# ComparativeGenomicsToolkit/paffy

Hardware: AMD Instinct MI355X
Metric: PAF records/sec (shatter+invert+trim pipe); % HBM roofline at 1/2/4/8 GPU (higher is better)
Workload: dtype u8/int64 (float32 identity predicate); 1 GPU; cfg3: 10M synthetic PAF records, mean 2k cigar ops, invert | trim | shatter; pipe=invert|trim|shatter, pipeline_contexts=2, stream_records=10000000, mean_cigar_ops=2048

## Files before the change

paffy_amd/csrc/flat_kernel.h:

```cpp
#ifndef PAFFY_FLAT_KERNEL_H_
#define PAFFY_FLAT_KERNEL_H_

#define FLAT_TILE 1024u
#define FLAT_TILE_SHIFT 10u
#define FLAT_CHUNK_PIECES 4u
#define FLAT_P_CAP 512u
#define FLAT_NO_CHUNK 0xffffffffu
#define FLAT_F_IRREG 1u
#define FLAT_F_NONPLAIN 2u

struct PieceSum {
    uint32_t cnt;
    uint32_t m, x;
    uint32_t ins, del;
    uint32_t rows;
    uint32_t extra;
    uint32_t text_end;
};
static_assert(sizeof(PieceSum) == 32, "two 16-byte stores");

struct FlatParams {
    const uint8_t *in;
    uint32_t in_len;
    const RecMeta *meta;
    const uint32_t *chunk_rec;
    uint32_t n_chunk_slots;
    const uint16_t *nd;
    PieceSum *sums;
    uint32_t *ops_mirror;
    DevInfo *info;
    uint32_t items_mode;
};

__device__ __forceinline__ uint32_t nondigit16(const uint4 &v) {
    const uint32_t w[4] = {v.x, v.y, v.z, v.w};
    uint32_t m = 0;
#pragma unroll
    for (int j = 0; j < 4; j++) {
        uint32_t nd = nondigit4(w[j]) >> 7;
        nd = (nd | (nd >> 7) | (nd >> 14) | (nd >> 21)) & 0xfu;
        m |= nd << (4 * j);
    }
    return m;
}
__device__ __forceinline__ uint32_t wave_fold_u32(uint32_t x) {
    x += dpp_mov_u32<DPP_ROW_SHR(1), 0xf, 0xf>(x);
    x += dpp_mov_u32<DPP_ROW_SHR(2), 0xf, 0xf>(x);
    x += dpp_mov_u32<DPP_ROW_SHR(4), 0xf, 0xf>(x);
    x += dpp_mov_u32<DPP_ROW_SHR(8), 0xf, 0xf>(x);
    x += dpp_mov_u32<DPP_BCAST15, 0xa, 0xf>(x);
    x += dpp_mov_u32<DPP_BCAST31, 0xc, 0xf>(x);
    return x;
}
__device__ __forceinline__ uint32_t wave_sum_u32(uint32_t v) { return wave_last_u32(wave_fold_u32(v)); }
__device__ __forceinline__ void wave_sum6_u32(uint32_t (&x)[6]) {
#define FLAT_FOLD_STEP(CTRL, RM)                                                  \
    _Pragma("unroll") for (int k = 0; k < 6; k++) x[k] += dpp_mov_u32<CTRL, RM, 0xf>(x[k]);
    FLAT_FOLD_STEP(DPP_ROW_SHR(1), 0xf)
    FLAT_FOLD_STEP(DPP_ROW_SHR(2), 0xf)
    FLAT_FOLD_STEP(DPP_ROW_SHR(4), 0xf)
    FLAT_FOLD_STEP(DPP_ROW_SHR(8), 0xf)
    FLAT_FOLD_STEP(DPP_BCAST15, 0xa)
    FLAT_FOLD_STEP(DPP_BCAST31, 0xc)
#undef FLAT_FOLD_STEP
#pragma unroll
    for (int k = 0; k < 6; k++) x[k] = wave_last_u32(x[k]);
}
__device__ __forceinline__ uint32_t uni(uint32_t x) { return (uint32_t)__builtin_amdgcn_readfirstlane((int)x); }
__device__ __forceinline__ uint32_t lane_val(uint32_t x, uint32_t l) { return (uint32_t)__builtin_amdgcn_readlane((int)x, (int)l); }

#define FLAT_PARSE_LDS (16u + FLAT_TILE + 2u * FLAT_P_CAP)
#define FLAT_PARSE_WAVES 4u
template <uint32_t MODE>
__global__ __launch_bounds__(64 * FLAT_PARSE_WAVES) void k_flat_parse(FlatParams F) {
    __shared__ __attribute__((aligned(16))) uint8_t smem[FLAT_PARSE_WAVES][FLAT_PARSE_LDS];
    const uint32_t lane = threadIdx.x & 63u, wave = uni(threadIdx.x >> 6);
    uint8_t *T = smem[wave];
    uint16_t *Pl = reinterpret_cast<uint16_t *>(T + 16u + FLAT_TILE);
    const uint32_t n_waves = gridDim.x * FLAT_PARSE_WAVES;
    for (uint32_t c = blockIdx.x * FLAT_PARSE_WAVES + wave; c < F.n_chunk_slots; c += n_waves) {
        const uint32_t rec = F.chunk_rec[c];
        if (rec == FLAT_NO_CHUNK) continue;
        const uint32_t cg_off = F.meta[rec].cg_off, cg_end = cg_off + F.meta[rec].cg_len;
        const uint32_t tile_first = cg_off >> FLAT_TILE_SHIFT;
        const uint32_t np = ((cg_end - 1u) >> FLAT_TILE_SHIFT) - tile_first + 1u;
        const uint32_t p0 = (c - ((tile_first >> 2) + rec)) * FLAT_CHUNK_PIECES, p1 = p0 + FLAT_CHUNK_PIECES < np ? p0 + FLAT_CHUNK_PIECES : np;
        PieceSum *const rec_sums = F.sums + (tile_first + rec);
        uint32_t tile = tile_first + p0;
        __builtin_amdgcn_wave_barrier();
        if (lane == 0) {
            uint4 h = make_uint4(0, 0, 0, 0);
            if (tile > 0) h = *reinterpret_cast<const uint4 *>(F.in + ((size_t)tile << FLAT_TILE_SHIFT) - 16u);
            *reinterpret_cast<uint4 *>(T) = h;
        }
        __builtin_amdgcn_wave_barrier();
        uint32_t n = 0;
        int32_t prev;
        uint32_t text_end = 0;
        if (p0 == 0) {
            prev = (int32_t)cg_off - 1 - (int32_t)(tile << FLAT_TILE_SHIFT);
        } else {
            uint32_t cnt = 0;
            {
                const uint32_t g = (tile_first << FLAT_TILE_SHIFT) + lane * 16u;
                uint4 v = make_uint4(0x30303030u, 0x30303030u, 0x30303030u, 0x30303030u);
                if (g < F.in_len) v = *reinterpret_cast<const uint4 *>(F.in + g);
                const uint32_t lo_b = cg_off > g ? (cg_off - g < 16u ? cg_off - g : 16u) : 0u;
                cnt = (uint32_t)__popc(nondigit16(v) & 0xffffu & ~((1u << lo_b) - 1u));
            }
            for (uint32_t t = tile_first + 1u + lane; t < tile; t += 64u) cnt += F.nd[t];
            n = wave_sum_u32(cnt);
            const uint4 h = *reinterpret_cast<const uint4 *>(T);
            const uint32_t hm = nondigit16(h);
            prev = hm ? (int32_t)(31 - __clz((int)hm)) - 16 : -17;
            text_end = (uint32_t)((int32_t)(tile << FLAT_TILE_SHIFT) + prev + 1 - (int32_t)cg_off);
        }
        uint16_t *dst = reinterpret_cast<uint16_t *>(F.ops_mirror + (cg_off >> 1));
        for (uint32_t p = p0; p < p1; p++, tile++) {
            const uint32_t t0 = tile << FLAT_TILE_SHIFT, g = t0 + lane * 16u;
            uint4 v = make_uint4(0, 0, 0, 0);
            if (g < F.in_len) v = *reinterpret_cast<const uint4 *>(F.in + g);
            *reinterpret_cast<uint4 *>(T + 16u + lane * 16u) = v;
            const uint32_t ndm = nondigit16(v);
            const uint32_t lo_b = cg_off > g ? (cg_off - g < 16u ? cg_off - g : 16u) : 0u;
            const uint32_t hi_b = cg_end < g + 16u ? (cg_end > g ? cg_end - g : 0u) : 16u;
            uint32_t opmask = ndm & (hi_b >= 16u ? 0xffffu : ((1u << hi_b) - 1u)) & ~((1u << lo_b) - 1u);
            uint32_t bad = (hi_b > lo_b && g + hi_b == cg_end && !((ndm >> (hi_b - 1u)) & 1u)) ? 1u : 0u;
            const uint32_t cnt = (uint32_t)__popc(opmask), inc = wave_incl_scan_u32(cnt), total = wave_last_u32(inc);
            uint32_t rank = inc - cnt;
            while (opmask) {
                const uint32_t j = (uint32_t)__ffs((int)opmask) - 1u;
                opmask &= opmask - 1u;
                if (rank < FLAT_P_CAP) Pl[rank] = (uint16_t)(lane * 16u + j);
                rank++;
            }
            if (total > FLAT_P_CAP) bad = 1u;
            __builtin_amdgcn_wave_barrier();
            const uint32_t top = total < FLAT_P_CAP ? total : FLAT_P_CAP;
            uint32_t acc_mx = 0, acc_id = 0, acc_re = 0, nonplain = 0;
            uint32_t before_first = (uint32_t)prev;
            for (uint32_t i = lane; i < top; i += 64u) {
                const uint32_t pos = Pl[i];
                const uint32_t before = (uint32_t)__builtin_amdgcn_update_dpp((int)before_first, (int)pos, 0x138 , 0xf, 0xf, false);
                before_first = lane_val(pos, 63);
                const uint32_t k = pos - before - 1u;
                const uint32_t a = 12u + pos, sh = a & 3u;
                const uint32_t *wp = reinterpret_cast<const uint32_t *>(T + (a - sh));
                const uint32_t d0 = wp[0], d1 = wp[1];
                const uint32_t hi = __builtin_amdgcn_alignbyte(d1, d0, sh);
                const uint32_t ch = (d1 >> (8u * sh)) & 0xffu;
                const uint32_t kk = k < 4u ? k : 4u;
                const uint32_t x = kk ? ((hi ^ 0x30303030u) & (0xffffffffu << (32u - 8u * kk))) : 0u;
                const uint32_t pr = ((x << 3) + (x << 1) + (x >> 8)) & 0x00ff00ffu;
                const uint32_t len = __umul24(pr & 0xffu, 100u) + (pr >> 16);
                const uint32_t dl = ch - 0x3du;
                const bool known = dl < 28u && ((0x08011081u >> dl) & 1u);
                const uint32_t code = (0x04001023u >> (dl & 0x1cu)) & 7u;
                const bool lead0 = kk >= 2u && ((hi >> (8u * (4u - kk))) & 0xffu) == (uint32_t)'0';
                bad |= ((k - 1u > 3u) | (len - 1u >= 8191u) | lead0 | !known) ? 1u : 0u;
                dst[n + i] = (uint16_t)((len << 3) | code);
                const uint32_t l16 = len & 0xffffu;
                acc_mx += l16 << (((0x16u >> code) & 1u) << 4);
                acc_id += (code == (uint32_t)OP_I ? l16 : 0u) + (code == (uint32_t)OP_D ? l16 << 16 : 0u);
                if (MODE == 2u) acc_re += (code == (uint32_t)OP_M ? 1u : 0u) + (code == (uint32_t)OP_I ? 1u << 16 : 0u);
                else acc_re += code == (uint32_t)OP_M ? 1u + ((MODE == 1u ? (len + 15u) >> 4 : kk - 1u) << 16) : 0u;
                nonplain |= code > (uint32_t)OP_D ? 1u : 0u;
            }
            uint32_t sums6[6] = {acc_mx & 0xffffu, acc_mx >> 16, acc_id & 0xffffu, acc_id >> 16, acc_re & 0xffffu, acc_re >> 16};
            wave_sum6_u32(sums6);
            const uint32_t s_m = sums6[0], s_x = sums6[1], s_i = sums6[2], s_d = sums6[3], s_r = sums6[4], s_e = sums6[5];
            const uint32_t flags = (__any(bad != 0) ? FLAT_F_IRREG : 0u) | (__any(nonplain != 0) ? FLAT_F_NONPLAIN : 0u);
            if (total) {
                const int32_t last = (int32_t)Pl[top - 1u];
                text_end = t0 + (uint32_t)last + 1u - cg_off;
                prev = last - (int32_t)FLAT_TILE;
            } else {
                prev -= (int32_t)FLAT_TILE;
                if (prev < -64) prev = -64;
            }
            if (lane == 0) {
                uint4 *o = reinterpret_cast<uint4 *>(rec_sums + p);
                o[0] = make_uint4(total | (flags << 16), s_m, s_x, s_i);
                o[1] = make_uint4(s_d, s_r, s_e, text_end);
            }
            n += total;
            __builtin_amdgcn_wave_barrier();
            if (lane == 63u) *reinterpret_cast<uint4 *>(T) = v;
            __builtin_amdgcn_wave_barrier();
        }
    }
}


struct FlatSizeParams {
    KParams P;
    PieceSum *sums;
    uint8_t *flat_done;
    uint32_t *defer;
};

struct FlatPre {
    uint32_t cnt, m, x, ins, del, rows, extra, text;
};
__device__ __forceinline__ FlatPre flat_sub(const FlatPre &a, const FlatPre &b) {
    FlatPre r;
    r.cnt = a.cnt - b.cnt; r.m = a.m - b.m; r.x = a.x - b.x; r.ins = a.ins - b.ins; r.del = a.del - b.del;
    r.rows = a.rows - b.rows; r.extra = a.extra - b.extra; r.text = a.text - b.text;
    return r;
}
__device__ __forceinline__ uint32_t flat_ld(const uint32_t *p) { return __hip_atomic_load(p, __ATOMIC_RELAXED, __HIP_MEMORY_SCOPE_AGENT); }

struct FlatRec {
    const PieceSum *ps;
    uint32_t np, n_ops;
    bool in_regs;
    FlatPre inc;
    const uint16_t *ops;
    bool want_text;
    bool extra_icount;

    __device__ __forceinline__ FlatPre piece_prefix(uint32_t j) const {
        FlatPre r;
        r.cnt = r.m = r.x = r.ins = r.del = r.rows = r.extra = r.text = 0;
        if (j == 0) return r;
        if (in_regs) {
            const uint32_t l = j - 1u;
            r.cnt = lane_val(inc.cnt, l); r.m = lane_val(inc.m, l); r.x = lane_val(inc.x, l); r.ins = lane_val(inc.ins, l);
            r.del = lane_val(inc.del, l); r.rows = lane_val(inc.rows, l); r.extra = lane_val(inc.extra, l); r.text = lane_val(inc.text, l);
        } else {
            const uint32_t *q = reinterpret_cast<const uint32_t *>(ps + (j - 1u));
            r.cnt = uni(flat_ld(q)); r.m = uni(flat_ld(q + 1)); r.x = uni(flat_ld(q + 2)); r.ins = uni(flat_ld(q + 3));
            r.del = uni(flat_ld(q + 4)); r.rows = uni(flat_ld(q + 5)); r.extra = uni(flat_ld(q + 6)); r.text = uni(flat_ld(q + 7));
        }
        return r;
    }
    __device__ __forceinline__ uint32_t piece_of(uint32_t r) const {
        if (in_regs) {
            const uint32_t lane = threadIdx.x & 63u;
            return (uint32_t)__popcll(__ballot(lane < np && inc.cnt <= r));
        }
        uint32_t lo = 0, hi = np;
        while (lo < hi) {
            const uint32_t mid = (lo + hi) >> 1;
            if (uni(flat_ld(&ps[mid].cnt)) <= r) lo = mid + 1u;
            else hi = mid;
        }
        return lo;
    }
    __device__ __forceinline__ FlatPre raw_prefix(uint32_t r) const {
        if (r >= n_ops) return piece_prefix(np);
        const uint32_t pc = piece_of(r);
        FlatPre a = piece_prefix(pc);
        if (a.cnt == r) return a;
        const uint32_t lane = threadIdx.x & 63u;
        uint32_t sm = 0, sx = 0, si = 0, sd = 0, sr = 0, se = 0, st = 0;
        for (uint32_t i = a.cnt + lane; i < r; i += 64u) {
            const uint32_t w = ops[i], len = w >> 3, code = w & 7u;
            const uint32_t is_m = 0u - ((0x9u >> code) & 1u);
            const uint32_t dg = (len >= 10u) + (len >= 100u) + (len >= 1000u);
            sm += len & is_m;
            sx += len & ~is_m;
            si += code == (uint32_t)OP_I ? len : 0u;
            sd += code == (uint32_t)OP_D ? len : 0u;
            sr += code == (uint32_t)OP_M ? 1u : 0u;
            se += extra_icount ? (code == (uint32_t)OP_I ? 1u : 0u) : (code == (uint32_t)OP_M ? dg : 0u);
            st += dg + 2u;
        }
        uint32_t sums6[6] = {sm, sx, si, sd, sr, se};
        wave_sum6_u32(sums6);
        a.m += sums6[0]; a.x += sums6[1]; a.ins += sums6[2]; a.del += sums6[3];
        a.rows += sums6[4]; a.extra += sums6[5];
        if (want_text) a.text += wave_sum_u32(st);
        a.cnt = r;
        return a;
    }
};

struct FlatView {
    uint32_t lo, n;
    bool rev, swp;
    FlatPre wlo, whi;
    uint32_t cut_m = 0, cut_x = 0;
    __device__ __forceinline__ uint32_t tm() const { return whi.m - wlo.m - cut_m; }
    __device__ __forceinline__ uint32_t tx() const { return whi.x - wlo.x - cut_x; }
    __device__ __forceinline__ uint32_t ins_v() const { return swp ? whi.del - wlo.del : whi.ins - wlo.ins; }
    __device__ __forceinline__ uint32_t del_v() const { return swp ? whi.ins - wlo.ins : whi.del - wlo.del; }
    __device__ __forceinline__ int64_t tq() const { return (int64_t)tm() + (int64_t)tx() - (int64_t)del_v(); }
    __device__ __forceinline__ int64_t tt() const { return (int64_t)tm() + (int64_t)tx() - (int64_t)ins_v(); }
};

struct FlatState {
    int64_t qlen, qs, qe, tlen, ts, te;
    bool same;
};
__device__ __forceinline__ void flat_invert(FlatState &s) {
    int64_t t;
    t = s.qs; s.qs = s.ts; s.ts = t;
    t = s.qe; s.qe = s.te; s.te = t;
    t = s.qlen; s.qlen = s.tlen; s.tlen = t;
}
__device__ __forceinline__ int flat_check(const FlatState &s, const FlatView &v) {
    if (s.qs < 0 || s.qs >= s.qlen) return PAFFY_ERR_CHECK_QSTART;
    if (s.qs > s.qe || s.qe > s.qlen) return PAFFY_ERR_CHECK_QEND;
    if (s.ts < 0 || s.ts >= s.tlen) return PAFFY_ERR_CHECK_TSTART;
    if (s.ts > s.te || s.te > s.tlen) return PAFFY_ERR_CHECK_TEND;
    if (v.tq() != s.qe - s.qs) return PAFFY_ERR_CHECK_CIGAR_Q;
    if (v.tt() != s.te - s.ts) return PAFFY_ERR_CHECK_CIGAR_T;
    return 0;
}

__device__ __forceinline__ bool flat_filter_pass(const KParams &P, const RecMeta &m, const FlatView &v) {
    const int64_t mm = v.tm(), mx = v.tx();
    const int64_t all = mm + mx;
    const int64_t ins = all - v.tt(), del = all - v.tq();
    const double identity = ratio_f32(mm, mm + (mx - ins - del));
    const double identity_with_gaps = ratio_f32(mm, all);
    const int64_t f_as = P.filter.min_alignment_score, f_cs = P.filter.min_chain_score, f_tl = P.filter.max_tile_level;
    const double f_id = P.filter.min_identity, f_idg = P.filter.min_identity_with_gaps;
    return m.score >= f_as && m.chain_score >= f_cs && (f_tl == -1 || m.tile_level <= f_tl) && identity >= f_id && identity_with_gaps >= f_idg;
}
__device__ __forceinline__ void flat_dropped(const KParams &P, uint8_t *flat_done, uint32_t rec) {
    RecPlan *dp = static_cast<RecPlan *>(P.rec_plan) + rec;
    flat_done[rec] = 1;
    P.status[rec] = (uint32_t)KLASS_LDS << 16;
    P.err_aux[rec] = 0;
    P.n_ops[rec] = 0;
    P.out_len[rec] = 0;
    P.out_rows[rec] = 0;
    dp->flags = 128u;
    dp->n = 0;
}

__device__ __forceinline__ void flat_stats(const KParams &P, uint32_t rec, const FlatView &v) {
    const uint32_t n_i = v.whi.extra - v.wlo.extra, n_other = (v.whi.cnt - v.wlo.cnt) - (v.whi.rows - v.wlo.rows);
    const uint32_t n_d = n_other - n_i;
    int64_t *o = P.rec_stats + 6ull * rec;
    o[0] = (int64_t)v.tm();
    o[1] = (int64_t)v.tx() - (int64_t)(v.whi.ins - v.wlo.ins) - (int64_t)(v.whi.del - v.wlo.del);
    o[2] = (int64_t)(v.swp ? n_d : n_i);
    o[3] = (int64_t)(v.swp ? n_i : n_d);
    o[4] = (int64_t)v.ins_v();
    o[5] = (int64_t)v.del_v();
}
__device__ __forceinline__ bool flat_ratio_lt(uint32_t num, uint32_t den, float thr_f, double thr) {
    const float nf = __uint2float_rn(num), df = __uint2float_rn(den);
    const float p = __fmul_rn(thr_f, df);
    if (nf < __fmul_rn(p, 0.999996f)) return true;
    if (nf > __fmul_rn(p, 1.000004f)) return false;
    return (double)__fdiv_rn(nf, df) < thr;
}
__device__ __forceinline__ bool flat_ratio_ge(uint32_t num, uint32_t den, float id_f, double idd) {
    const float nf = __uint2float_rn(num), df = __uint2float_rn(den);
    const float p = __fmul_rn(id_f, df);
    if (nf > __fmul_rn(p, 1.000004f)) return true;
    if (nf < __fmul_rn(p, 0.999996f)) return false;
    return (double)__fdiv_rn(nf, df) >= idd;
}

__device__ __forceinline__ void flat_trim_prefix(const FlatRec &R, FlatState &s, FlatView &v, float thr_f, float id_f, int64_t max_trim) {
    const double thr = (double)thr_f, idd = (double)id_f;
    const uint32_t lane = threadIdx.x & 63u;
    const uint32_t w_end = v.lo + v.n;
    const uint32_t nb = (R.np + 63u) >> 6;
    int32_t trim_idx = -1;
    uint32_t hit_m = 0, hit_x = 0;
    for (uint32_t bi = 0; bi < nb && trim_idx < 0; bi++) {
        const uint32_t b = v.rev ? bi : nb - 1u - bi;
        const uint32_t p = b * 64u + lane;
        uint32_t a_cnt = 0, a_m = 0, a_x = 0, b_cnt = 0, b_m = 0, b_x = 0;
        if (p < R.np) {
            if (R.in_regs) {
                b_cnt = R.inc.cnt; b_m = R.inc.m; b_x = R.inc.x;
            } else {
                const uint32_t *q = reinterpret_cast<const uint32_t *>(R.ps + p);
                b_cnt = flat_ld(q); b_m = flat_ld(q + 1); b_x = flat_ld(q + 2);
            }
        }
        if (R.in_regs) {
            a_cnt = dpp_mov_u32<0x138, 0xf, 0xf>(b_cnt); a_m = dpp_mov_u32<0x138, 0xf, 0xf>(b_m); a_x = dpp_mov_u32<0x138, 0xf, 0xf>(b_x);
        } else if (p > 0 && p < R.np) {
            const uint32_t *q = reinterpret_cast<const uint32_t *>(R.ps + (p - 1u));
            a_cnt = flat_ld(q); a_m = flat_ld(q + 1); a_x = flat_ld(q + 2);
        }
        if (a_cnt < v.lo) { a_cnt = v.lo; a_m = v.wlo.m; a_x = v.wlo.x; }
        if (a_cnt > w_end) { a_cnt = w_end; a_m = v.whi.m; a_x = v.whi.x; }
        if (b_cnt < v.lo) { b_cnt = v.lo; b_m = v.wlo.m; b_x = v.wlo.x; }
        if (b_cnt > w_end) { b_cnt = w_end; b_m = v.whi.m; b_x = v.whi.x; }
        const bool live = p < R.np && b_cnt > a_cnt;
        const uint32_t c_m = v.rev ? v.whi.m - b_m : a_m - v.wlo.m, c_x = v.rev ? v.whi.x - b_x : a_x - v.wlo.x;
        const uint32_t chunk_x = b_x - a_x;
        const bool may_hit = live && !(c_m > 0 && (double)c_m >= thr * 1.00001 * (double)(c_m + c_x + chunk_x)) &&
                             !(max_trim >= 0 && (int64_t)c_m + (int64_t)c_x > max_trim);
        unsigned long long flagged = __ballot(may_hit);
        while (flagged) {
            const uint32_t t = v.rev ? (uint32_t)__ffsll((long long)flagged) - 1u : 63u - (uint32_t)__clzll((long long)flagged);
            flagged &= ~(1ull << t);
            const uint32_t ra = lane_val(a_cnt, t), rb = lane_val(b_cnt, t);
            uint32_t pm = lane_val(c_m, t), px = lane_val(c_x, t);
            const uint32_t x_end = px + lane_val(chunk_x, t);
            const uint32_t vb = v.rev ? w_end - rb : ra - v.lo, ve = v.rev ? w_end - ra : rb - v.lo;
            int32_t hit = -1;
            for (uint32_t i0 = vb; i0 < ve; i0 += 64u) {
                if (i0 != vb && pm > 0 && (double)pm >= thr * 1.00001 * (double)(pm + x_end)) break;
                const uint32_t i = i0 + lane;
                uint32_t len = 0, code = 0;
                if (i < ve) {
                    const uint32_t w = R.ops[v.rev ? w_end - 1u - i : v.lo + i];
                    len = w >> 3;
                    code = w & 7u;
                }
                const uint32_t is_m = 0u - ((0x9u >> code) & 1u);
                const uint32_t im = wave_incl_scan_u32(len & is_m), ix = wave_incl_scan_u32(len & ~is_m);
                const uint32_t cm = pm + im, cx = px + ix;
                const bool ok = i < ve && !(max_trim >= 0 && (int64_t)(cm + cx) > max_trim) && flat_ratio_lt(cm, cm + cx, thr_f, thr);
                const unsigned long long hb = __ballot(ok);
                if (hb) {
                    const uint32_t hl = 63u - (uint32_t)__clzll((long long)hb);
                    hit = (int32_t)(i0 + hl);
                    hit_m = lane_val(cm, hl);
                    hit_x = lane_val(cx, hl);
                }
                pm += wave_last_u32(im);
                px += wave_last_u32(ix);
            }
            if (hit >= 0) {
                trim_idx = hit;
                break;
            }
        }
    }
    if (trim_idx < 0) return;
    uint32_t best = 0xffffffffu;
    {
        uint32_t pm = 0, px = 0;
        for (uint32_t i0 = 0; i0 <= (uint32_t)trim_idx && best == 0xffffffffu; i0 += 64u) {
            const uint32_t i = i0 + lane;
            uint32_t len = 0, code = 0;
            if (i <= (uint32_t)trim_idx) {
                const uint32_t w = R.ops[v.rev ? w_end - 1u - i : v.lo + i];
                len = w >> 3;
                code = w & 7u;
            }
            const uint32_t is_m = 0u - ((0x9u >> code) & 1u);
            const uint32_t vm = len & is_m, vx = len & ~is_m;
            const uint32_t im = wave_incl_scan_u32(vm), ix = wave_incl_scan_u32(vx);
            const uint32_t sm = hit_m - (pm + im - vm), sx = hit_x - (px + ix - vx);
            const bool ok = i <= (uint32_t)trim_idx && flat_ratio_ge(sm, sm + sx, id_f, idd);
            const unsigned long long hb = __ballot(ok);
            if (hb) best = i0 + (uint32_t)__ffsll((long long)hb) - 1u;
            pm += wave_last_u32(im);
            px += wave_last_u32(ix);
        }
    }
    const uint32_t count = best != 0xffffffffu ? best : (uint32_t)trim_idx + 1u;
    if (count == 0) return;
    const int64_t old_tt = v.tt(), old_tq = v.tq();
    {
        const FlatPre cut = R.raw_prefix(v.rev ? v.lo + v.n - count : v.lo + count);
        if (v.rev) {
            v.whi = cut;
        } else {
            v.wlo = cut;
            v.lo += count;
        }
    }
    v.n -= count;
    const int64_t d_t = old_tt - v.tt(), d_q = old_tq - v.tq();
    s.ts += d_t;
    if (s.same) s.qs += d_q;
    else s.qe -= d_q;
}

#define FLAT_F_ROW_PIECES 0x200000u
#define FLAT_F_COPY 0x400000u
#define FLAT_COPY_MAX (1u << 18)
#define FLAT_ROW_PIECES_BYTES 144u
struct LanePieceSink {
    uint32_t (*S)[256];
// ... 941 lines not shown
```

Before: 24.79 million records/s.

## Parse CIGAR tile with per-step ballots instead of LDS position list

Replaces the two-pass parse (scatter op positions into an LDS list, then re-read them per lane) with a single pass over 128-byte steps. Each lane examines two bytes, uses ballots and mbcnt to rank op terminators, and reads the preceding digit word directly from the tile in LDS. Lengths are decoded with udot4 and op length is inferred from leading non-digits. This removes the serial ffs loop and the LDS position buffer, at the cost of more intricate edge handling for capped tiles and adjacent ops, and it recomputes the last-op position from ballot masks.

```diff
diff --git a/paffy_amd/csrc/flat_kernel.h b/paffy_amd/csrc/flat_kernel.h
--- a/paffy_amd/csrc/flat_kernel.h
+++ b/paffy_amd/csrc/flat_kernel.h
@@ -69,14 +69,21 @@
 __device__ __forceinline__ uint32_t uni(uint32_t x) { return (uint32_t)__builtin_amdgcn_readfirstlane((int)x); }
 __device__ __forceinline__ uint32_t lane_val(uint32_t x, uint32_t l) { return (uint32_t)__builtin_amdgcn_readlane((int)x, (int)l); }
 
-#define FLAT_PARSE_LDS (16u + FLAT_TILE + 2u * FLAT_P_CAP)
+#define FLAT_PARSE_LDS (16u + FLAT_TILE)
 #define FLAT_PARSE_WAVES 4u
+#define FLAT_STEP 128u
+__device__ __forceinline__ uint64_t lanes_below(uint32_t n) { return n >= 64u ? ~0ull : (1ull << n) - 1ull; }
+__device__ __forceinline__ bool lane_bit(uint64_t m) { return __builtin_amdgcn_inverse_ballot_w64(m); }
+__device__ __forceinline__ uint32_t lanes_before(uint64_t m, uint32_t add) {
+    return __builtin_amdgcn_mbcnt_hi((uint32_t)(m >> 32), __builtin_amdgcn_mbcnt_lo((uint32_t)m, add));
+}
 template <uint32_t MODE>
 __global__ __launch_bounds__(64 * FLAT_PARSE_WAVES) void k_flat_parse(FlatParams F) {
     __shared__ __attribute__((aligned(16))) uint8_t smem[FLAT_PARSE_WAVES][FLAT_PARSE_LDS];
     const uint32_t lane = threadIdx.x & 63u, wave = uni(threadIdx.x >> 6);
     uint8_t *T = smem[wave];
-    uint16_t *Pl = reinterpret_cast<uint16_t *>(T + 16u + FLAT_TILE);
+    const uint32_t *lw = reinterpret_cast<const uint32_t *>(T + 8u + (lane >> 1) * 4u);
+    const uint32_t o8 = (lane & 1u) * 16u;
     const uint32_t n_waves = gridDim.x * FLAT_PARSE_WAVES;
     for (uint32_t c = blockIdx.x * FLAT_PARSE_WAVES + wave; c < F.n_chunk_slots; c += n_waves) {
         const uint32_t rec = F.chunk_rec[c];
@@ -97,6 +104,7 @@
         uint32_t n = 0;
         int32_t prev;
         uint32_t text_end = 0;
+        bool capped = false;
         if (p0 == 0) {
             prev = (int32_t)cg_off - 1 - (int32_t)(tile << FLAT_TILE_SHIFT);
         } else {
@@ -121,59 +129,101 @@
             uint4 v = make_uint4(0, 0, 0, 0);
             if (g < F.in_len) v = *reinterpret_cast<const uint4 *>(F.in + g);
             *reinterpret_cast<uint4 *>(T + 16u + lane * 16u) = v;
-            const uint32_t ndm = nondigit16(v);
-            const uint32_t lo_b = cg_off > g ? (cg_off - g < 16u ? cg_off - g : 16u) : 0u;
-            const uint32_t hi_b = cg_end < g + 16u ? (cg_end > g ? cg_end - g : 0u) : 16u;
-            uint32_t opmask = ndm & (hi_b >= 16u ? 0xffffu : ((1u << hi_b) - 1u)) & ~((1u << lo_b) - 1u);
-            uint32_t bad = (hi_b > lo_b && g + hi_b == cg_end && !((ndm >> (hi_b - 1u)) & 1u)) ? 1u : 0u;
-            const uint32_t cnt = (uint32_t)__popc(opmask), inc = wave_incl_scan_u32(cnt), total = wave_last_u32(inc);
-            uint32_t rank = inc - cnt;
-            while (opmask) {
-                const uint32_t j = (uint32_t)__ffs((int)opmask) - 1u;
-                opmask &= opmask - 1u;
-                if (rank < FLAT_P_CAP) Pl[rank] = (uint16_t)(lane * 16u + j);
-                rank++;
+            __builtin_amdgcn_wave_barrier();
+            const uint32_t lo = cg_off > t0 ? cg_off - t0 : 0u, hi = cg_end - t0 < FLAT_TILE ? cg_end - t0 : FLAT_TILE;
+            uint32_t bad = 0;
+            if (cg_end - t0 <= FLAT_TILE && hi > lo) bad = (uint32_t)T[16u + hi - 1u] - (uint32_t)'0' <= 9u ? 1u : 0u;
+            uint16_t *const dst_t = dst + n;
+            uint32_t acc_mx = 0, acc_id = 0, acc_re = 0, nonplain = 0;
+            uint32_t total = 0;
+            int32_t last = 0;
+            uint64_t e0 = 0, e1 = 0;
+            uint32_t eb = 0;
+#pragma unroll
+            for (uint32_t s = 0; s < FLAT_TILE / FLAT_STEP; s++) {
+                const uint32_t sb = s * FLAT_STEP;
+                if (hi <= sb || lo >= sb + FLAT_STEP) continue;
+                uint64_t in0 = ~0ull, in1 = ~0ull;
+                if (lo > sb || hi < sb + FLAT_STEP) {
+                    const uint32_t a = lo > sb ? lo - sb : 0u, b = hi - sb < FLAT_STEP ? hi - sb : FLAT_STEP;
+                    in0 = lanes_below((b + 1u) >> 1) & ~lanes_below((a + 1u) >> 1);
+                    in1 = lanes_below(b >> 1) & ~lanes_below(a >> 1);
+                }
+                const uint32_t w0 = lw[s * (FLAT_STEP / 4u)], w1 = lw[s * (FLAT_STEP / 4u) + 1u], w2 = lw[s * (FLAT_STEP / 4u) + 2u];
+                const uint32_t c0 = (w2 >> o8) & 0xffu, c1 = (w2 >> (o8 + 8u)) & 0xffu;
+                const uint64_t l0 = __ballot(c0 - (uint32_t)'0' > 9u) & in0, l1 = __ballot(c1 - (uint32_t)'0' > 9u) & in1;
+                const uint64_t any = l0 | l1, both = l0 & l1;
+                if (any == 0) continue;
+                const uint32_t cnt = (uint32_t)__popcll(l0) + (uint32_t)__popcll(l1);
+                const uint32_t rank = lanes_before(l0, lanes_before(l1, 0u));
+                const uint32_t room = FLAT_P_CAP - (total < FLAT_P_CAP ? total : FLAT_P_CAP);
+                uint16_t *const dst_s = dst_t + total;
+                const bool first = lane_bit(l0);
+                const uint32_t sh8 = first ? o8 : o8 + 8u;
+                const uint32_t num = __builtin_amdgcn_alignbit(w2, w1, sh8);
+                const uint32_t ch = (w2 >> sh8) & 0xffu;
+                const uint32_t c5 = (__builtin_amdgcn_alignbyte(w1, w0, 3u) >> sh8) & 0xffu;
+                uint32_t k8 = (uint32_t)__clz((int)nondigit4(num));
+                bool bad_k = k8 == 0u || (k8 == 32u && c5 - (uint32_t)'0' <= 9u);
+                if (capped) {
+                    if (lane_bit(any) && rank == 0u) {
+                        const uint32_t k = (uint32_t)((int32_t)(sb + 2u * lane + (first ? 0u : 1u)) - prev - 1);
+                        k8 = k < 4u ? 8u * k : 32u;
+                        bad_k = k - 1u > 3u;
+                    }
+                    capped = false;
+                }
+                if (lane_bit(any) && rank < room) {
+                    const uint32_t x = k8 ? ((num ^ 0x30303030u) & (0xffffffffu << (32u - k8))) : 0u;
+                    const uint32_t len = __builtin_amdgcn_udot4(x, 0x010a0000u, __umul24(__builtin_amdgcn_udot4(x, 0x0000010au, 0u, false), 100u), false);
+                    const uint32_t dl = ch - 0x3du;
+                    const bool known = dl < 28u && ((0x08011081u >> dl) & 1u);
+                    const uint32_t code = (0x04001023u >> (dl & 0x1cu)) & 7u;
+                    const bool lead0 = k8 >= 16u && ((num >> (32u - k8)) & 0xffu) == (uint32_t)'0';
+                    bad |= (bad_k | (len - 1u >= 8191u) | lead0 | !known) ? 1u : 0u;
+                    dst_s[rank] = (uint16_t)((len << 3) | code);
+                    const uint32_t l16 = len & 0xffffu;
+                    acc_mx += l16 << (((0x16u >> code) & 1u) << 4);
+                    acc_id += (code == (uint32_t)OP_I ? l16 : 0u) + (code == (uint32_t)OP_D ? l16 << 16 : 0u);
+                    if (MODE == 2u) acc_re += (code == (uint32_t)OP_M ? 1u : 0u) + (code == (uint32_t)OP_I ? 1u << 16 : 0u);
+                    else acc_re += code == (uint32_t)OP_M ? 1u + ((MODE == 1u ? (len + 15u) >> 4 : (k8 >> 3) - 1u) << 16) : 0u;
+                    nonplain |= code > (uint32_t)OP_D ? 1u : 0u;
+                }
+                if (both) {
+                    if (lane_bit(both)) {
+                        bad = 1u;
+                        if (rank + 1u < room) {
+                            const uint32_t dl = c1 - 0x3du;
+                            const uint32_t code = (0x04001023u >> (dl & 0x1cu)) & 7u;
+                            dst_s[rank + 1u] = (uint16_t)code;
+                            if (MODE == 2u) acc_re += (code == (uint32_t)OP_M ? 1u : 0u) + (code == (uint32_t)OP_I ? 1u << 16 : 0u);
+                            else acc_re += code == (uint32_t)OP_M ? 1u + ((MODE == 1u ? 0u : 0u - 1u) << 16) : 0u;
+                            nonplain |= code > (uint32_t)OP_D ? 1u : 0u;
+                        }
+                    }
+                }
+                if (cnt <= room) {
+                    e0 = l0; e1 = l1; eb = sb;
+                } else if (room) {
+                    e0 = __ballot(lane_bit(l0) && rank == room - 1u);
+                    e1 = __ballot((lane_bit(both) ? rank + 1u : lane_bit(l0) ? ~0u : rank) == room - 1u) & l1;
+                    eb = sb;
+                }
+                total += cnt;
             }
             if (total > FLAT_P_CAP) bad = 1u;
-            __builtin_amdgcn_wave_barrier();
-            const uint32_t top = total < FLAT_P_CAP ? total : FLAT_P_CAP;
-            uint32_t acc_mx = 0, acc_id = 0, acc_re = 0, nonplain = 0;
-            uint32_t before_first = (uint32_t)prev;
-            for (uint32_t i = lane; i < top; i += 64u) {
-                const uint32_t pos = Pl[i];
-                const uint32_t before = (uint32_t)__builtin_amdgcn_update_dpp((int)before_first, (int)pos, 0x138 , 0xf, 0xf, false);
-                before_first = lane_val(pos, 63);
-                const uint32_t k = pos - before - 1u;
-                const uint32_t a = 12u + pos, sh = a & 3u;
-                const uint32_t *wp = reinterpret_cast<const uint32_t *>(T + (a - sh));
-                const uint32_t d0 = wp[0], d1 = wp[1];
-                const uint32_t hi = __builtin_amdgcn_alignbyte(d1, d0, sh);
-                const uint32_t ch = (d1 >> (8u * sh)) & 0xffu;
-                const uint32_t kk = k < 4u ? k : 4u;
-                const uint32_t x = kk ? ((hi ^ 0x30303030u) & (0xffffffffu << (32u - 8u * kk))) : 0u;
-                const uint32_t pr = ((x << 3) + (x << 1) + (x >> 8)) & 0x00ff00ffu;
-                const uint32_t len = __umul24(pr & 0xffu, 100u) + (pr >> 16);
-                const uint32_t dl = ch - 0x3du;
-                const bool known = dl < 28u && ((0x08011081u >> dl) & 1u);
-                const uint32_t code = (0x04001023u >> (dl & 0x1cu)) & 7u;
-                const bool lead0 = kk >= 2u && ((hi >> (8u * (4u - kk))) & 0xffu) == (uint32_t)'0';
-                bad |= ((k - 1u > 3u) | (len - 1u >= 8191u) | lead0 | !known) ? 1u : 0u;
-                dst[n + i] = (uint16_t)((len << 3) | code);
-                const uint32_t l16 = len & 0xffffu;
-                acc_mx += l16 << (((0x16u >> code) & 1u) << 4);
-                acc_id += (code == (uint32_t)OP_I ? l16 : 0u) + (code == (uint32_t)OP_D ? l16 << 16 : 0u);
-                if (MODE == 2u) acc_re += (code == (uint32_t)OP_M ? 1u : 0u) + (code == (uint32_t)OP_I ? 1u << 16 : 0u);
-                else acc_re += code == (uint32_t)OP_M ? 1u + ((MODE == 1u ? (len + 15u) >> 4 : kk - 1u) << 16) : 0u;
-                nonplain |= code > (uint32_t)OP_D ? 1u : 0u;
+            {
+                const int32_t h0 = e0 ? 126 - 2 * (int32_t)__builtin_clzll(e0) : -1, h1 = e1 ? 127 - 2 * (int32_t)__builtin_clzll(e1) : -1;
+                last = (int32_t)eb + (h0 > h1 ? h0 : h1);
             }
             uint32_t sums6[6] = {acc_mx & 0xffffu, acc_mx >> 16, acc_id & 0xffffu, acc_id >> 16, acc_re & 0xffffu, acc_re >> 16};
             wave_sum6_u32(sums6);
             const uint32_t s_m = sums6[0], s_x = sums6[1], s_i = sums6[2], s_d = sums6[3], s_r = sums6[4], s_e = sums6[5];
             const uint32_t flags = (__any(bad != 0) ? FLAT_F_IRREG : 0u) | (__any(nonplain != 0) ? FLAT_F_NONPLAIN : 0u);
             if (total) {
-                const int32_t last = (int32_t)Pl[top - 1u];
                 text_end = t0 + (uint32_t)last + 1u - cg_off;
                 prev = last - (int32_t)FLAT_TILE;
+                capped = total > FLAT_P_CAP;
             } else {
                 prev -= (int32_t)FLAT_TILE;
                 if (prev < -64) prev = -64;
```

Result: slower. 23.40 million records/s (-5.6%).
